# actionml/universal-recommender

Hardware: AMD Instinct MI355X
Metric: cooccurrence pairs/sec (A'A+A'B) + LLR top-k items/sec (higher is better)
Workload: dtype int32 counts / f64 LLR; 1 GPU; config4: synthetic 10M users x 2M items, Zipf-1.0, 5 event types (purchase/view/add-to-cart/search/category-pref); generator=torch Philox on the GPU (universal_recommender_amd.synth.generate_device), maxEventsPerEventType=500, maxCorrelatorsPerEventType=50, seed=20260925, entry_point=urcco_context_build_device (C ABI, include/urcco.h), launch=one process per GPU, parallelism=items range-partitioned over 1 GPU(s), one HIP stream per event type

## Files before the change

universal-recommender_amd/_lib.py:

```python
from __future__ import annotations

import ctypes as C
import os
from typing import Optional

_HERE = os.path.dirname(os.path.abspath(__file__))
DEFAULT_PATH = os.path.join(_HERE, "lib", "liburcco.so")

OK, BAD_ARG, OOM_HOST, OOM_DEVICE, HIP_ERROR, INTERNAL, NO_DEVICE, RCCL_ERROR, BUSY = range(9)
FLAG_SINGLE_STREAM = 1
FLAG_FORCE_EXCHANGE = 2
FLAG_UNORDERED_ROWS = 4
FLAG_EMULATE_RANKS = 8
UNIQUE_ID_BYTES = 128
ROW_RATE_MAHOUT_INT_DIV = 0
ROW_RATE_FRACTIONAL = 1
RNG_SPLITMIX53 = 0
RNG_MIX32 = 0x100
N_STAGES = 17
N_BINS = 7
STATS_LEN = 32
REC_MAX_CLAUSES = 16
REC_MAX_NUM = 256
REC_NO_BACKFILL = 1
# ... 4 lines not shown
REC_WEIGHT_MAX = 1 << 20
EVAL_MAX_KS = 8
EVAL_TREE_BLOCK = 256
HIST_STATS_LEN = 8
REC_LDS_LIMIT = 3072
EXCH_SIZES = 4
DBG_GATHER_ONLY = 1
DBG_NO_LLR = 2
DBG_NO_TOPK = 4
DBG_NO_SELECT = 8
DBG_NO_RANK = 16
DBG_NO_COUNT_GATHER = 512
DBG_UNFUSED_EXPAND = 4096
DBG_GATHERED_PRIMARY = 8192
DBG_UNFILTERED_EXCHANGE = 16384
DBG_SELECT_DELAY = 131072
DBG_UNPACKED_COUNTS = 1048576
DBG_NO_PREFILTER = 8388608
DBG_COUNT_SCORED = 16777216
DBG_NO_DIRECT_RANK = 33554432
DBG_COUNT_DIRECT = 67108864
DBG_NO_SMALL_WAVE = 134217728
DBG_COUNT_SMALL_WAVE = 268435456
DBG_ROW_KERNELS = DBG_GATHER_ONLY | DBG_NO_LLR | DBG_NO_TOPK | DBG_NO_SELECT | DBG_NO_RANK | DBG_NO_COUNT_GATHER | DBG_SELECT_DELAY
STAGE_NAMES = ["column_counts", "downsample_flags", "downsample_scan", "downsample_compact", "transpose", "row_work", "binning",
               "entropy", "cco_rows_micro", "cco_rows_wave", "cco_rows_block_small", "cco_rows_block", "cco_rows_cu_half", "cco_rows_cu", "cco_rows_global", "compact_indicators", "exchange"]


class UrccoError(RuntimeError):
    def __init__(self, status: int, message: str):
        super().__init__(f"liburcco: {message} (status {status})")
        self.status = status


class Csr(C.Structure):
    _fields_ = [("n_rows", C.c_int64), ("n_cols", C.c_int64), ("row_ptr", C.c_void_p), ("col_idx", C.c_void_p)]


class Dataset(C.Structure):
    _fields_ = [("matrix", Csr), ("max_elements_per_row", C.c_int32), ("max_interesting_elements", C.c_int32),
                ("min_llr", C.c_double), ("has_min_llr", C.c_int32), ("reserved", C.c_int32)]


class Options(C.Structure):
    _fields_ = [("device", C.c_int32), ("row_rate_mode", C.c_int32), ("n_gpus", C.c_int32), ("flags", C.c_int32), ("reserved", C.c_int32 * 4)]

# ... 198 lines not shown
```

universal-recommender_amd/csrc/cco_kernels.h:

```cpp
#pragma once
#include <hip/hip_runtime.h>
#include <stdint.h>

namespace urcco {

constexpr int NBINS = 7;
constexpr int MP_KMAX_HOST = 256;

constexpr int SCAN_TILE = 2048;
constexpr int DS_TILE = 4096;
constexpr int GLOBAL_BIN_BLOCKS = 128;
constexpr int BIN_TILE = 1024;
constexpr int XLX_TABLE_HOST = 4096;
constexpr int BIN_COLS_HOST = 3 * NBINS + 5;
constexpr int BIN_OFF_LEN = NBINS + 5;
constexpr int CAND_SLOTS = 64;
constexpr int STATS_LEN = 32;

constexpr int32_t DBG_GATHER_ONLY = 1;
constexpr int32_t DBG_NO_LLR = 2;
constexpr int32_t DBG_NO_TOPK = 4;
constexpr int32_t DBG_NO_SELECT = 8;
constexpr int32_t DBG_NO_RANK = 16;
constexpr int32_t DBG_NO_COUNT_GATHER = 512;
constexpr int32_t DBG_UNFUSED_EXPAND = 4096;
constexpr int32_t DBG_GATHERED_PRIMARY = 8192;
constexpr int32_t DBG_UNFILTERED_EXCHANGE = 16384;
constexpr int32_t DBG_SELECT_DELAY = 131072;
constexpr int32_t DBG_UNPACKED_COUNTS = 1048576;
constexpr int32_t DBG_NO_PREFILTER = 8388608;
constexpr int32_t DBG_COUNT_SCORED = 16777216;
constexpr int32_t DBG_NO_DIRECT_RANK = 33554432;
constexpr int32_t DBG_COUNT_DIRECT = 67108864;
constexpr int32_t DBG_NO_SMALL_WAVE = 134217728;
constexpr int32_t DBG_COUNT_SMALL_WAVE = 268435456;
constexpr int32_t DBG_ROW_KERNELS = DBG_GATHER_ONLY | DBG_NO_LLR | DBG_NO_TOPK | DBG_NO_SELECT | DBG_NO_RANK | DBG_NO_COUNT_GATHER | DBG_SELECT_DELAY;

constexpr int32_t FORM_WIDE = 1;
constexpr int32_t FORM_PS64 = 2;
constexpr int32_t FORM_TILE = 4;
constexpr int32_t FORM_PACK = 8;
constexpr int32_t FORM_HOST = 16;
constexpr unsigned long long NARROW_LIMIT = 1ull << 32;
struct ExpandForm {
  int32_t* word;
  const int32_t* pack_bad;
  int32_t host_wide;
  int32_t host_narrow;
  unsigned long long limit;
  long long seed;
};

struct CcoArgs {
  const int32_t* bin_rows;
  const int32_t* bin_off;
  const int64_t* a_col_ptr;
  const unsigned* pstart32;
  const int64_t* wp;
// ... 264 lines not shown
```

universal-recommender_amd/csrc/cco_rows.hip:

```cpp
#include "cco_kernels.h"

#include <atomic>
#include <cstdlib>

#include "cco_common.h"
#include "cco_device.h"
#include "cco_select.h"


namespace urcco {

constexpr int E0 = 1024, E1S = 4096, E1 = 8192, E2S = 16384, E2 = 32768;
constexpr int MP_KMAX = 256;

__host__ __device__ constexpr int table_slots(int E, int T) { return (2 * E / 3) / (2 * T) * (2 * T); }
constexpr int URCCO_WB1 = 512;
constexpr int URCCO_WB2 = 8192;
__device__ __forceinline__ int choose_bin(long long w, long long ca, int32_t n_cols_b, int32_t count_bits, int32_t k) {
  if (ca <= 0 || w <= 0) return -1;
  if (count_bits < 31 && ca > ((1ll << count_bits) - 1)) return NBINS - 1;
  if (w <= 64 && ca <= 64) return 0;
  int cap_bin = NBINS - 1;
  const long long dmax = (w < (long long)n_cols_b ? w : (long long)n_cols_b) * 3 + (long long)k * 3 + 2;
  if (dmax <= E0) cap_bin = 1;
  else if (dmax <= E1S) cap_bin = 2;
  else if (dmax <= E1) cap_bin = 3;
  else if (dmax <= E2S) cap_bin = 4;
  else if (dmax <= E2) cap_bin = 5;
  const int work_bin = w <= URCCO_WB1 ? 1 : (w <= URCCO_WB2 ? 2 : 4);
  return cap_bin > work_bin ? cap_bin : work_bin;
}

constexpr int MICRO_SUBS = 3;
constexpr int SMALL_SUBS = 2;
constexpr int SMALL_P0 = 2, SMALL_P1 = 4;
constexpr int SMALL_KMAX = WAVE - 1;
static_assert(SMALL_KMAX + 1 <= WAVE && SMALL_KMAX >= 1, "k + 1 survivors (a self pair among them) must fit the lanes of the fast tail");
constexpr int IBINS = NBINS - 1 + MICRO_SUBS + SMALL_SUBS;
constexpr int SPLIT_MICRO = 1, SPLIT_SMALL = 2;
__device__ __forceinline__ int micro_sub(long long w, long long ca) { return (w <= 16 && ca <= 16) ? 0 : ((w <= 32 && ca <= 32) ? 1 : 2); }
__device__ __forceinline__ int small_sub(long long w, long long ca) { return ca > WAVE ? 2 : (w <= SMALL_P0 * WAVE ? 0 : (w <= SMALL_P1 * WAVE ? 1 : 2)); }
__device__ __forceinline__ int internal_bin(int b, long long w, long long ca, int split) {
  if (b < 0) return -1;
  if (b == 0) return (split & SPLIT_MICRO) ? micro_sub(w, ca) : MICRO_SUBS - 1;
  if (b == 1) return MICRO_SUBS + ((split & SPLIT_SMALL) ? small_sub(w, ca) : SMALL_SUBS);
  return b + MICRO_SUBS - 1 + SMALL_SUBS;
}
static bool micro_split_for(int32_t n_rows) {
  static const long long min_rows = [] { const char* e = getenv("URCCO_MICRO_SPLIT_ROWS"); return e && *e ? atoll(e) : 1000000ll; }();
  return (long long)n_rows >= min_rows;
}
__host__ __device__ constexpr int internal_off_index(int ib) {
  return ib == 0 ? 0 : (ib < MICRO_SUBS ? NBINS + ib : (ib == MICRO_SUBS ? 1 : (ib <= MICRO_SUBS + SMALL_SUBS ? NBINS + ib - 1 : ib - (MICRO_SUBS - 1 + SMALL_SUBS))));
}
static_assert(internal_off_index(MICRO_SUBS + 1) == NBINS + 3 && internal_off_index(MICRO_SUBS + 2) == NBINS + 4 && internal_off_index(MICRO_SUBS + 3) == 2 &&
              internal_off_index(IBINS - 1) == NBINS - 1, "bin_off layout");
__device__ __forceinline__ int internal_start(const int32_t* __restrict__ bin_off, int ib) { return bin_off[internal_off_index(ib)]; }
constexpr int BIN_THREADS = 256;
constexpr int BIN_ITEMS = BIN_TILE / BIN_THREADS;
constexpr int BIN_COLS = IBINS + 2 * NBINS + 1;
static_assert(BIN_COLS == BIN_COLS_HOST && BIN_OFF_LEN == NBINS + MICRO_SUBS + SMALL_SUBS, "scratch sizes of the callers");

__global__ __launch_bounds__(BIN_THREADS) void bin_count_kernel(int32_t item_lo, int32_t n, const int64_t* __restrict__ work,
                                                                const int32_t* __restrict__ cnt_a, int32_t n_cols_b, int32_t count_bits, int32_t k,
                                                                int64_t* __restrict__ tile_counts, int split) {
  __shared__ long long s_acc[BIN_COLS];
  if (threadIdx.x < BIN_COLS) s_acc[threadIdx.x] = 0;
  __syncthreads();
  int c[IBINS];
  long long pw[NBINS], pu[NBINS];
#pragma unroll
  for (int k = 0; k < IBINS; ++k) c[k] = 0;
#pragma unroll
  for (int k = 0; k < NBINS; ++k) { pw[k] = 0; pu[k] = 0; }
  long long pairs = 0;
#pragma unroll
  for (int q = 0; q < BIN_ITEMS; ++q) {
    const int64_t t = (int64_t)blockIdx.x * BIN_TILE + (int64_t)threadIdx.x * BIN_ITEMS + q;
    if (t < n) {
      const long long w = work[t];
      const long long ca = cnt_a[item_lo + t];
      pairs += w;
      const int b = choose_bin(w, ca, n_cols_b, count_bits, k);
      const int ib = internal_bin(b, w, ca, split);
// ... 54 lines not shown
#pragma unroll
      for (int d = 1; d < WAVE; d <<= 1) {
        const long long o = shfl_up_i64(inc, d);
        if (lane >= d) inc += o;
      }
      if (i < n_tiles) tile_counts[i * BIN_COLS + k] = carry + inc - v;
      carry += shfl_i64(inc, WAVE - 1);
    }
    if (lane == 0) s_tot[k] = carry;
  }
  __syncthreads();
  if (threadIdx.x == 0) {
    int32_t off = 0;
    for (int ib = 0; ib < IBINS; ++ib) {
      bin_off[internal_off_index(ib)] = off;
      off += (int32_t)s_tot[ib];
    }
    bin_off[NBINS] = off;
    if (stats) {
      for (int k = 0; k < NBINS; ++k) {
        long long rows = 0;
        if (k == 0) for (int q = 0; q < MICRO_SUBS; ++q) rows += s_tot[q];
        else if (k == 1) for (int q = 0; q <= SMALL_SUBS; ++q) rows += s_tot[MICRO_SUBS + q];
        else rows = s_tot[k + MICRO_SUBS - 1 + SMALL_SUBS];
        stats[1 + k] = rows;
        stats[1 + NBINS + k] = s_tot[IBINS + k];
        stats[1 + 2 * NBINS + k] = s_tot[IBINS + NBINS + k];
      }
      stats[0] = s_tot[IBINS + 2 * NBINS];
      stats[STATS_LEN - 1] = s_tot[0] + s_tot[1];
    }
  }
}

__global__ __launch_bounds__(BIN_THREADS) void bin_scatter_kernel(int32_t item_lo, int32_t n, const int64_t* __restrict__ work,
                                                                  const int32_t* __restrict__ cnt_a, int32_t n_cols_b, int32_t count_bits, int32_t k,
                                                                  const int64_t* __restrict__ tile_counts, const int32_t* __restrict__ bin_off,
                                                                  int32_t* __restrict__ bin_rows, int split) {
  __shared__ long long s_wave[SCAN_THREADS / WAVE];
  int b[BIN_ITEMS];
#pragma unroll
  for (int q = 0; q < BIN_ITEMS; ++q) {
    const int64_t t = (int64_t)blockIdx.x * BIN_TILE + (int64_t)threadIdx.x * BIN_ITEMS + q;
    b[q] = -1;
    if (t < n) {
      const long long w = work[t], ca = cnt_a[item_lo + t];
      b[q] = internal_bin(choose_bin(w, ca, n_cols_b, count_bits, k), w, ca, split);
// ... 384 lines not shown
  __shared__ unsigned long long s_runk[MP ? 2 * MP_KMAX : 1];
  __shared__ unsigned s_runc[MP ? 2 * MP_KMAX : 1];

  const int team = TEAMS == 1 ? 0 : uni((int)threadIdx.x / T);
  const int tl = threadIdx.x % T;
  const int lane = threadIdx.x & (WAVE - 1);
  unsigned* tab = s_tab + team * E;
  unsigned* cand = tab + SH;
  unsigned long long* share = s_share + (SHARE ? team * SHARE_WORDS : 0);
  PS* ustart = reinterpret_cast<PS*>(SHARE ? reinterpret_cast<long long*>(share) : s_ustart + team * T);
  unsigned* uoff = SHARE ? reinterpret_cast<unsigned*>(share + T) : s_uoff + team * (T + 1);
  unsigned* hist = SHARE ? reinterpret_cast<unsigned*>(share) : s_hist + team * NH * 128;
  unsigned* sel_res = s_selres + team * 4;
  unsigned* nsel = sel_res + 3;
  unsigned short* lst = SHARE ? reinterpret_cast<unsigned short*>(share) + SH_LST / 2 : s_lst + team * (SEL_CAP > 0 ? SEL_CAP : 1);
  unsigned long long* amb_key = SHARE ? share : s_ambkey + team * SEL_M;
  unsigned* amb_col = SHARE ? reinterpret_cast<unsigned*>(share + SEL_M) : s_ambcol + team * SEL_M;
  unsigned long long* sel_thr = s_selthr + team * 2;
  constexpr bool PF = PK && !MP && prefilter_class(T, E);
  static_assert(!PF || !SHARE || T == WAVE || (sizeof(PS) == 4 && T * 4 + PF_BINS * 2 <= T * 8), "the histogram sits behind the 32-bit starts");
  unsigned* pfh = (SHARE && T != WAVE) ? reinterpret_cast<unsigned*>(share) + T : hist;
  constexpr unsigned DL = PF ? direct_limit(T, E) : 0u;
  static_assert(DL <= (unsigned)SEL_M, "a directly ranked row lives in the ambiguous-set arrays");
  const int list_start = (T == WAVE && PK && !MP && (bin_arg & 2048)) ? a.bin_off[NBINS + MICRO_SUBS - 1 + SMALL_SUBS] : a.bin_off[bin];
  const int list_n = a.bin_off[bin + 1] - list_start;
  const int total_teams = gridDim.x * TEAMS;
  bool ident =(long long)a.n_cols_b * 3 + (long long)a.k * 3 + 2 <= E && a.n_cols_b <= SH;
  int cb = a.count_bits;
  unsigned cmask = (1u << cb) - 1u;
  unsigned long long cand_acc = 0ull;
  const double xlx_n = *a.xlx_n;
  const bool use16 = *a.cnt16_bad == 0;

  int li = blockIdx.x * TEAMS + team;
  if (li >= list_n) return;
  const int S = total_teams;
  auto pos_of = [&](int l) { return list_start + (l < list_n ? l : list_n - 1); };
  const unsigned* wp32 = reinterpret_cast<const unsigned*>(a.wp);
  const PS* pstart;
  if constexpr (PK) pstart = a.pstart32;
  else pstart = a.pstart64;
  const int lane3 = lane < 3 ? lane : 2;
  int idv = a.bin_rows[pos_of(li + lane3 * S)];
  int64_t cs_c, ce_c;
  int64_t bnd_b;
  {
    const int id0 = (int)wave_read_lane((unsigned)idv, 0);
// ... 887 lines not shown
        cand[rank] = rc;
        kkm[rank] = rk;
      }
      wave_sync();
      settle_prefetch();
      if ((unsigned)sl < n_out) {
        out_idx[obase + sl] = (int)cand[sl];
        out_llr[obase + sl] = __longlong_as_double((long long)kkm[sl]);
      }
      if (sl == 0 && live) out_count[i - a.item_lo] = (int)n_out;
    } else {
      settle_prefetch();
    }
    i_cur = i_n1;
    i_n1 = i_n2;
    i_n2 = i_n3;
    cs1 = cs2;
    ce1 = ce2;
    wave_sync();
  }
  if (a.cand && lane == 0 && cand_acc != 0ull) atomicAdd(&a.cand[(blockIdx.x * TEAMS + team) & (CAND_SLOTS - 1)], cand_acc);
}

constexpr int SMALL_TW = 512, SMALL_LOG2TW = 9;
constexpr int SMALL_LIST = WAVE + 4;
constexpr int SMALL_WORDS = 2 * SMALL_TW;
constexpr int SMALL_FACTOR = 4;
static_assert(2 * SMALL_P1 * WAVE <= SMALL_TW && SMALL_P1 * WAVE + 2 <= SMALL_TW && 3 * SMALL_LIST <= SMALL_TW / 2 && PF_BINS / 2 <= SMALL_TW / 2, "accumulator load <= 1/2; the marks and the fallback's keys fit the phase region, its staged words and columns the accumulator");
static_assert(PF_BINS / 2 + 2 * WAVE + 3 * SMALL_LIST <= SMALL_TW && (PF_BINS / 2 + 2 * WAVE + SMALL_LIST) % 2 == 0, "fast tail arrays; 64-bit keys 8-byte aligned");
template <int P>
__global__ __launch_bounds__(256, URCCO_OCC_MICRO) void cco_rows_small_kernel(CcoArgs a, int flags) {
  if (!(a.b_packed != nullptr && (a.pk_known != 0 || *a.form == 0))) return;
  static_assert(P == SMALL_P0 || P == SMALL_P1, "one instantiation per sub-list");
  const int32_t* bin_rows = a.bin_rows;
  const int64_t* a_col_ptr = a.a_col_ptr;
  const unsigned* pstart = a.pstart32;
  const int32_t* b_col_idx = a.b_packed;
  const int cshift = 32 - a.count_bits;
  const unsigned colmask = (1u << cshift) - 1u;
  const int32_t* cnt_a = a.cnt_a;
  const double* ent_a = a.ent_a;
  const double* xlx_tab = a.xlx_tab;
  const double* xlx_hi = a.xlx_hi;
  const double* col_ent = a.col_ent;
  int32_t* out_idx = a.out_idx;
  double* out_llr = a.out_llr;
  int32_t* out_count = a.out_count;
  const long long n_users = a.n_users;
  const bool has_pf = a.pf_limit != nullptr;
  const unsigned short* lim_tab = has_pf ? a.pf_limit : reinterpret_cast<const unsigned short*>(a.cnt_a);
  constexpr int TEAMS = 256 / WAVE;
  __shared__ __attribute__((aligned(16))) unsigned s_tab[TEAMS * SMALL_WORDS];
  const int team = threadIdx.x / WAVE;
  const int lane = threadIdx.x & (WAVE - 1);
  unsigned* tab = s_tab + team * SMALL_WORDS;
  unsigned* marks = tab + SMALL_TW;
  unsigned* pfh = marks;
  unsigned* st_v = marks + PF_BINS / 2;
  unsigned* st_c = st_v + WAVE;
  unsigned* cand = st_c + WAVE;
  unsigned long long* kkm = reinterpret_cast<unsigned long long*>(cand + SMALL_LIST);
  unsigned long long* fkeys = reinterpret_cast<unsigned long long*>(marks);
  const int list_start = P == SMALL_P0 ? a.bin_off[1] : a.bin_off[NBINS + 3];
  const int list_n = (P == SMALL_P0 ? a.bin_off[NBINS + 3] : a.bin_off[NBINS + 4]) - list_start;
  const int total_teams = gridDim.x * TEAMS;
  const bool ident = a.n_cols_b <= SMALL_TW;
  const int cb = a.count_bits;
  const unsigned cmask = (1u << cb) - 1u;
  const double xlx_n = __longlong_as_double((long long)uni((int64_t)__double_as_longlong(*a.xlx_n)));
  const unsigned pf_need = (unsigned)a.k + (a.exclude_self ? 1u : 0u);
  unsigned long long cand_acc = 0ull;

  int li = blockIdx.x * TEAMS + team;
  if (li >= list_n) return;
  const int stride = total_teams;
  auto pos_of = [&](int l) { return list_start + (l < list_n ? l : list_n - 1); };
  const unsigned* wp32 = reinterpret_cast<const unsigned*>(a.wp);
  const int lane3 = lane < 3 ? lane : 2;
  int idv = bin_rows[pos_of(li + lane3 * stride)];
  int64_t bnd_b;
  unsigned pf_w1, pf_wp, pf_start;
  int n_cur;
  {
    const int id0 = (int)wave_read_lane((unsigned)idv, 0);
    const int id1 = (int)wave_read_lane((unsigned)idv, 1);
    const int64_t cs0 = uni(a_col_ptr[id0]), ce0 = uni(a_col_ptr[id0 + 1]);
    bnd_b = a_col_ptr[id1 + (lane & 1)];
    n_cur = (int)(ce0 - cs0);
    const int64_t pl = lane < n_cur ? cs0 + lane : ce0 - 1;
    pf_w1 = wp32[ce0];
    pf_wp = wp32[pl];
    pf_start = pstart[pl];
  }
  URCCO_SETTLE(idv); URCCO_SETTLE(bnd_b); URCCO_SETTLE(pf_w1); URCCO_SETTLE(pf_wp); URCCO_SETTLE(pf_start);
#pragma unroll
  for (int q = 0; q < SMALL_TW / WAVE; ++q) tab[lane + q * WAVE] = 0u;
  int64_t bnd_c = 0;
  for (; li < list_n; li += stride, bnd_b = bnd_c) {
    const int i = (int)wave_read_lane((unsigned)idv, 0);
    const int id2 = (int)wave_read_lane((unsigned)idv, 2);
    const int64_t cs_n = wave_read_lane64(bnd_b, 0), ce_n = wave_read_lane64(bnd_b, 1);
    const unsigned w0 = wave_read_lane(pf_wp, 0);
    unsigned total = uni(pf_w1) - w0;
    if (total > (unsigned)(P * WAVE) || n_cur > WAVE) {
      if (lane == 0) atomicAdd(a.err, 1ull);
      total = 0u;
    }
    const bool owns_user = lane < n_cur;
    const unsigned my_off = owns_user ? pf_wp - w0 : total;
    const unsigned my_delta = (owns_user ? pf_start : 0u) - my_off;
    int lz = lane;
    URCCO_OPAQUE(lz);
    idv = bin_rows[pos_of(li + (1 + (lz < 3 ? lz : 2)) * stride)];
    bnd_c = a_col_ptr[id2 + (lz & 1)];
    int iv = i;
    URCCO_OPAQUE(iv);
    const int row_ca = cnt_a[iv];
    const double row_entropy = ent_a[iv];
    const unsigned row_lim = lim_tab[iv];
    n_cur = (int)(ce_n - cs_n);
    {
      const int64_t pl = lz < n_cur ? cs_n + lz : ce_n - 1;
      pf_w1 = wp32[ce_n];
      pf_wp = wp32[pl];
      pf_start = pstart[pl];
    }
#pragma unroll
    for (int r = 0; r < P; ++r) marks[lane + r * WAVE] = 0u;
    if (lane < 2) marks[P * WAVE + lane] = 0u;
    wave_sync();
    if (owns_user && my_off <= total) atomicMax(&marks[my_off], (unsigned)lane);
    wave_sync();
    unsigned jj[P];
    unsigned carry = 0u;
#pragma unroll
    for (int r = 0; r < P; ++r) {
      const unsigned m = wave_inclusive_max(marks[lane + r * WAVE]);
      const unsigned o = m > carry ? m : carry;
      carry = wave_read_lane(o, WAVE - 1);
      const unsigned base_o = wave_gather(my_delta, o);
      const unsigned t = (unsigned)(r * WAVE + lane);
      jj[r] = 0u;
      if (t < total) jj[r] = (unsigned)b_col_idx[base_o + t];
    }
    unsigned slot[P];
#pragma unroll
    for (int r = 0; r < P; ++r) {
      slot[r] = 0xffffffffu;
      if ((unsigned)(r * WAVE + lane) < total) {
        bool ok;
        slot[r] = tab_insert_claim(tab, (jj[r] & colmask) + 1u, cb, (unsigned)(SMALL_TW - 1), 32 - SMALL_LOG2TW, ident, &ok);
        if (!ok) atomicAdd(a.err, 1ull);
      }
    }
    wave_sync();
    unsigned vv[P];
    unsigned D = 0u;
#pragma unroll
    for (int r = 0; r < P; ++r) {
      const bool is_cand = slot[r] != 0xffffffffu;
      D += (unsigned)__popcll(__ballot(is_cand));
      vv[r] = 0u;
      if (is_cand) {
        vv[r] = tab[slot[r]];
        tab[slot[r]] = 0u;
      }
    }
    if (has_pf && D > pf_need) {
      unsigned zero = 0u;
      URCCO_OPAQUE(zero);
      *reinterpret_cast<uint2*>(&pfh[2 * lane]) = make_uint2(zero, zero);
      wave_sync();
#pragma unroll
      for (int r = 0; r < P; ++r)
        if (vv[r] != 0u) pf_count(pfh, vv[r] & cmask, jj[r] >> cshift);
      wave_sync();
      unsigned cstar, lim;
      if (pf_find_cut(pfh, lane, pf_need, row_lim, cstar, lim)) {
#pragma unroll
        for (int r = 0; r < P; ++r)
          if (pf_drops(vv[r] & cmask, jj[r] >> cshift, cstar, lim)) vv[r] = 0u;
      }
      wave_sync();
    }
    unsigned pos[P];
    unsigned n_surv = 0u;
#pragma unroll
    for (int r = 0; r < P; ++r) {
      const unsigned long long m = __ballot(vv[r] != 0u);
      pos[r] = n_surv + lanes_below(m);
      n_surv += (unsigned)__popcll(m);
    }
    if (!(flags & 4096)) cand_acc += (flags & 256) ? n_surv : D;
    else cand_acc += n_surv <= (unsigned)WAVE ? 1ull : (1ull << 32) + 1ull;
    const int64_t obase = ((int64_t)(i - a.item_lo)) * a.k;
    auto settle_prefetch = [&]() {
      URCCO_SETTLE(idv); URCCO_SETTLE(bnd_c); URCCO_SETTLE(pf_w1); URCCO_SETTLE(pf_wp); URCCO_SETTLE(pf_start);
    };
    const bool fast = n_surv <= (unsigned)WAVE;
    {
      unsigned* sv = fast ? st_v : tab;
      unsigned* sc = fast ? st_c : tab + SMALL_TW / 2;
#pragma unroll
      for (int r = 0; r < P; ++r)
        if (vv[r] != 0u) {
          sv[pos[r]] = vv[r];
          sc[pos[r]] = jj[r] >> cshift;
        }
    }
    unsigned* cand_l = cand;
    unsigned long long* kkm_l = kkm;
    unsigned n_list = n_surv;
    bool listed = true;
    unsigned long long mk = 0ull;
    int jc = 0;
    if (fast) {
      wave_sync();
      const bool is_cand = (unsigned)lane < n_surv;
      const unsigned v1 = is_cand ? st_v[lane] : 0u;
      const unsigned cbj = is_cand ? st_c[lane] : 0u;
      if (n_surv + (unsigned)lane < (unsigned)SMALL_LIST) {
        unsigned zero = 0u;
        URCCO_OPAQUE(zero);
        *reinterpret_cast<uint2*>(&kkm[n_surv + (unsigned)lane]) = make_uint2(zero, zero);
        cand[n_surv + (unsigned)lane] = 0xffffffffu;
      }
      jc = (int)(v1 >> cb) - 1;
      const long long k11 = (long long)(v1 & cmask);
      const bool in_tables = !is_cand || llr_operands_in_tables((unsigned)k11, (long long)row_ca, cbj, n_users, col_ent);
      const bool all_in_tables = __ballot(!in_tables) == 0ull;
      if (is_cand) {
        if (!(a.exclude_self && jc == i)) {
          const double llr = all_in_tables ? llr_from_tables(row_entropy, xlx_n, (unsigned)k11, (unsigned)row_ca, cbj, xlx_tab, xlx_hi, col_ent)
                                           : llr_of(row_entropy, xlx_n, k11, (long long)row_ca, (long long)cbj, n_users, xlx_tab, xlx_hi, col_ent);
          if (llr > 0.0 && (!a.has_min_llr || llr >= a.min_llr)) mk = (unsigned long long)__double_as_longlong(llr);
        }
        kkm[lane] = mk;
        cand[lane] = (unsigned)jc;
      }
      wave_sync();
    } else {
      unsigned* fcol = tab + SMALL_TW / 2;
      wave_sync();
      unsigned n_valid = 0u;
      unsigned long long kand = ~0ull, kor = 0ull;
#pragma unroll 1
      for (unsigned base = 0; base < n_surv; base += WAVE) {
        const unsigned x = base + (unsigned)lane;
        unsigned long long key = 0ull;
        if (x < n_surv) {
          const unsigned v1 = tab[x], cbj = fcol[x];
          const int j = (int)(v1 >> cb) - 1;
          const long long k11 = (long long)(v1 & cmask);
          if (!(a.exclude_self && j == i)) {
            const double llr = llr_operands_in_tables((unsigned)k11, (long long)row_ca, cbj, n_users, col_ent)
                                   ? llr_from_tables(row_entropy, xlx_n, (unsigned)k11, (unsigned)row_ca, cbj, xlx_tab, xlx_hi, col_ent)
                                   : llr_of(row_entropy, xlx_n, k11, (long long)row_ca, (long long)cbj, n_users, xlx_tab, xlx_hi, col_ent);
            if (llr > 0.0 && (!a.has_min_llr || llr >= a.min_llr)) key = (unsigned long long)__double_as_longlong(llr);
          }
          fkeys[x] = key;
          fcol[x] = (unsigned)j;
        }
        if (key != 0ull) {
          kand &= key;
          kor |= key;
// ... 109 lines not shown
        } else {
          rk = kkm_l[ln];
          rc = cand_l[ln];
          rank = rank_by_counting_strided<1>(kkm_l, cand_l, 0u, n_list, rk, rc);
        }
        wave_sync();
        const unsigned n_out = (unsigned)(n_valid < a.k ? n_valid : a.k);
        if ((unsigned)lane < n_list && rk != 0ull && rank < n_out) {
          cand_l[rank] = rc;
          kkm_l[rank] = rk;
        }
        wave_sync();
        settle_prefetch();
        if ((unsigned)lane < n_out) {
          out_idx[obase + lane] = (int)cand_l[lane];
          out_llr[obase + lane] = __longlong_as_double((long long)kkm_l[lane]);
        }
        if (lane == 0) out_count[i - a.item_lo] = (int)n_out;
      }
    }
    if (!fast) {
      wave_sync();
#pragma unroll
      for (int q = 0; q < SMALL_TW / WAVE; ++q) tab[lane + q * WAVE] = 0u;
    }
    wave_sync();
  }
  if (a.cand && cand_acc != 0ull && lanes_below(~0ull) == 0u) atomicAdd(&a.cand[blockIdx.x & (CAND_SLOTS - 1)], cand_acc);
}

constexpr int GB_THREADS = 1024;
constexpr int GSEL_K = 1024;

__device__ __forceinline__ int64_t g_start(const unsigned* ps32, const int64_t* ps64, bool nar, int64_t p) { return nar ? (int64_t)ps32[p] : ps64[p]; }
__device__ __forceinline__ int64_t g_len(const int64_t* wp, bool nar, int64_t p) {
  const unsigned* w = reinterpret_cast<const unsigned*>(wp);
  return nar ? (int64_t)(unsigned)(w[p + 1] - w[p]) : wp[p + 1] - wp[p];
}
__global__ __launch_bounds__(GB_THREADS) void cco_rows_global_kernel(CcoArgs a) {
  constexpr int NW = GB_THREADS / WAVE;
  __shared__ unsigned long long s_pkey[2][NW];
  __shared__ int s_pcol[2][NW];
  __shared__ int s_ncand;
  __shared__ SelScratch s_select;
  __shared__ int s_nsel;
  __shared__ unsigned long long s_selk[GSEL_K];
  __shared__ unsigned s_selc[GSEL_K];
// ... 166 lines not shown
template <int T, int E, int U, bool MP = false>
constexpr RowClass row_class(int factor) {
  return {T < 256 ? 256 : T, (T < 256 ? 256 : T) / T, factor, MP ? 0u : direct_limit(T, E),
          cco_rows_kernel<T, E, U, MP, true, false>, cco_rows_kernel<T, E, U, MP, false, true>, cco_rows_kernel<T, E, U, MP, false, false>};
}
constexpr RowClass ROW_CLASS[NBINS] = {{256, 4, 8, 0u, nullptr, nullptr, nullptr},
                                       row_class<64, E0, URCCO_U_WAVE>(8),         row_class<256, E1S, URCCO_U_BS>(8), row_class<256, E1, URCCO_U_B>(8),
                                       row_class<512, E2S, URCCO_U_H>(4),          row_class<1024, E2, URCCO_U_C>(4),  row_class<1024, E2, URCCO_U_C, true>(2)};
constexpr int MICRO_FACTOR32 = 3, MICRO_FACTOR16 = 2;

static int blocks_per_cu(int bin) {
  static std::atomic<int> cache[NBINS];
  if (cache[bin].load(std::memory_order_relaxed) == 0) {
    int n = 0;
    const hipError_t e = bin == 0 ? hipOccupancyMaxActiveBlocksPerMultiprocessor(&n, (cco_rows_micro_kernel<WAVE, false, false>), ROW_CLASS[0].block, 0)
                                  : hipOccupancyMaxActiveBlocksPerMultiprocessor(&n, ROW_CLASS[bin].plain, ROW_CLASS[bin].block, 0);
    cache[bin].store((e == hipSuccess && n > 0) ? n : 1, std::memory_order_relaxed);
  }
  return cache[bin].load(std::memory_order_relaxed);
}

hipError_t launch_cco_rows_bin(hipStream_t st, int n_cu, const CcoArgs& args, RowsPlan plan, int bin, int32_t n_rows) {
  const RowClass& c = ROW_CLASS[bin];
  auto grid = [&](int factor) {
    const long long fill = (long long)n_cu * blocks_per_cu(bin);
    long long cap = ((long long)n_rows + c.teams * 32 - 1) / (c.teams * 32);
    if (cap < 2 * fill) cap = 2 * fill;
    long long blocks = fill * factor;
    if (blocks > cap) blocks = cap;
    return dim3((unsigned)blocks);
  };
  const bool count_direct = (args.debug & DBG_COUNT_DIRECT) != 0, count_small = (args.debug & DBG_COUNT_SMALL_WAVE) != 0;
  CcoArgs pk = args, plain = args, small = args;
  if ((count_direct && c.direct == 0u) || count_small) pk.cand = nullptr;
  if (count_direct || count_small) plain.cand = nullptr;
  if (count_direct) small.cand = nullptr;
  const int pk_bits = ((args.debug & DBG_COUNT_SCORED) ? 256 : 0) | ((args.debug & DBG_NO_DIRECT_RANK) ? 512 : 0) | (count_direct ? 1024 : 0);
  auto enqueue = [&](auto dbg_kernel, auto pk_kernel, auto plain_kernel, int factor, auto... bin_arg) {
    if (plan == RowsPlan::DEBUG) hipLaunchKernelGGL(dbg_kernel, grid(factor), dim3(c.block), 0, st, plain, bin_arg...);
    if (plan_runs_pk(plan)) hipLaunchKernelGGL(pk_kernel, grid(factor), dim3(c.block), 0, st, pk, (bin_arg | pk_bits)...);
    if (plan_runs_plain(plan)) hipLaunchKernelGGL(plain_kernel, grid(factor), dim3(c.block), 0, st, plain, bin_arg...);
  };
  if (bin == 0) {
    enqueue(cco_rows_micro_kernel<64, true, false>, cco_rows_micro_kernel<64, false, true>, cco_rows_micro_kernel<64, false, false>, c.factor);
    if (micro_split_for(n_rows)) {
      enqueue(cco_rows_micro_kernel<32, true, false>, cco_rows_micro_kernel<32, false, true>, cco_rows_micro_kernel<32, false, false>, MICRO_FACTOR32);
      enqueue(cco_rows_micro_kernel<16, true, false>, cco_rows_micro_kernel<16, false, true>, cco_rows_micro_kernel<16, false, false>, MICRO_FACTOR16);
    }
  } else if (bin == NBINS - 1 && args.g_blocks > 0) {
    plain.b_packed = nullptr;
    hipLaunchKernelGGL(cco_rows_global_kernel, dim3((unsigned)args.g_blocks), dim3(GB_THREADS), 0, st, plain);
  } else if (bin == 1 && plan_runs_pk(plan) && micro_split_for(n_rows) && args.k <= SMALL_KMAX && !(args.debug & DBG_NO_SMALL_WAVE)) {
    const int small_bits = ((args.debug & DBG_COUNT_SCORED) ? 256 : 0) | (count_small ? 4096 : 0);
    hipLaunchKernelGGL(cco_rows_small_kernel<SMALL_P0>, grid(SMALL_FACTOR), dim3(c.block), 0, st, small, small_bits);
    hipLaunchKernelGGL(cco_rows_small_kernel<SMALL_P1>, grid(SMALL_FACTOR), dim3(c.block), 0, st, small, small_bits);
    hipLaunchKernelGGL(c.pk, grid(c.factor), dim3(c.block), 0, st, pk, bin | pk_bits | 2048);
    if (plan_runs_plain(plan)) hipLaunchKernelGGL(c.plain, grid(c.factor), dim3(c.block), 0, st, plain, bin);
  } else {
    enqueue(c.dbg, c.pk, c.plain, c.factor, bin);
  }
  return hipGetLastError();
}

__global__ __launch_bounds__(256) void bin_out_stats_kernel(const int32_t* __restrict__ bin_rows, const int32_t* __restrict__ bin_off,
                                                            int32_t item_lo, const int32_t* __restrict__ out_count, const unsigned long long* __restrict__ cand,
                                                            int64_t* __restrict__ stats) {
  __shared__ long long s_wave[SCAN_THREADS / WAVE];
  const int bin = blockIdx.x;
  if (bin == 0 && blockIdx.y == 0 && threadIdx.x == 0 && cand) {
    long long c = 0;
    for (int q = 0; q < CAND_SLOTS; ++q) c += (long long)cand[q];
    stats[2 + 4 * NBINS] = c;
  }
  long long v = 0;
  for (int t = bin_off[bin] + blockIdx.y * 256 + threadIdx.x; t < bin_off[bin + 1]; t += 256 * gridDim.y) v += out_count[bin_rows[t] - item_lo];
  long long tot;
  block_exclusive_scan(v, s_wave, &tot);
  if (threadIdx.x == 0 && tot) atomicAdd((unsigned long long*)&stats[1 + 3 * NBINS + bin], (unsigned long long)tot);
// ... 10 lines not shown
```

Measured before the change: 39.83 billion pairs/s.

## Route mid-size rows to a one-wave kernel with two users per lane

```diff
diff --git a/universal-recommender_amd/_lib.py b/universal-recommender_amd/_lib.py
--- a/universal-recommender_amd/_lib.py
+++ b/universal-recommender_amd/_lib.py
@@ -50,6 +50,8 @@
 DBG_COUNT_DIRECT = 67108864
 DBG_NO_SMALL_WAVE = 134217728
 DBG_COUNT_SMALL_WAVE = 268435456
+DBG_NO_BLOCK_SMALL_WAVE = 536870912
+DBG_COUNT_BLOCK_SMALL_WAVE = 1073741824
 DBG_ROW_KERNELS = DBG_GATHER_ONLY | DBG_NO_LLR | DBG_NO_TOPK | DBG_NO_SELECT | DBG_NO_RANK | DBG_NO_COUNT_GATHER | DBG_SELECT_DELAY
 STAGE_NAMES = ["column_counts", "downsample_flags", "downsample_scan", "downsample_compact", "transpose", "row_work", "binning",
                "entropy", "cco_rows_micro", "cco_rows_wave", "cco_rows_block_small", "cco_rows_block", "cco_rows_cu_half", "cco_rows_cu", "cco_rows_global", "compact_indicators", "exchange"]
diff --git a/universal-recommender_amd/csrc/cco_kernels.h b/universal-recommender_amd/csrc/cco_kernels.h
--- a/universal-recommender_amd/csrc/cco_kernels.h
+++ b/universal-recommender_amd/csrc/cco_kernels.h
@@ -12,8 +12,8 @@
 constexpr int GLOBAL_BIN_BLOCKS = 128;
 constexpr int BIN_TILE = 1024;
 constexpr int XLX_TABLE_HOST = 4096;
-constexpr int BIN_COLS_HOST = 3 * NBINS + 5;
-constexpr int BIN_OFF_LEN = NBINS + 5;
+constexpr int BIN_COLS_HOST = 3 * NBINS + 7;
+constexpr int BIN_OFF_LEN = NBINS + 7;
 constexpr int CAND_SLOTS = 64;
 constexpr int STATS_LEN = 32;
 
@@ -34,6 +34,8 @@
 constexpr int32_t DBG_COUNT_DIRECT = 67108864;
 constexpr int32_t DBG_NO_SMALL_WAVE = 134217728;
 constexpr int32_t DBG_COUNT_SMALL_WAVE = 268435456;
+constexpr int32_t DBG_NO_BLOCK_SMALL_WAVE = 536870912;
+constexpr int32_t DBG_COUNT_BLOCK_SMALL_WAVE = 1073741824;
 constexpr int32_t DBG_ROW_KERNELS = DBG_GATHER_ONLY | DBG_NO_LLR | DBG_NO_TOPK | DBG_NO_SELECT | DBG_NO_RANK | DBG_NO_COUNT_GATHER | DBG_SELECT_DELAY;
 
 constexpr int32_t FORM_WIDE = 1;
diff --git a/universal-recommender_amd/csrc/cco_rows.hip b/universal-recommender_amd/csrc/cco_rows.hip
--- a/universal-recommender_amd/csrc/cco_rows.hip
+++ b/universal-recommender_amd/csrc/cco_rows.hip
@@ -32,34 +32,48 @@
 }
 
 constexpr int MICRO_SUBS = 3;
-constexpr int SMALL_SUBS = 2;
-constexpr int SMALL_P0 = 2, SMALL_P1 = 4;
+constexpr int SMALL_SUBS = 3;
+constexpr int BLOCK_SUBS = 1;
+constexpr int SMALL_P0 = 2, SMALL_P1 = 4, SMALL_P2 = 8;
+constexpr int SMALL_U2 = 2;
 constexpr int SMALL_KMAX = WAVE - 1;
 static_assert(SMALL_KMAX + 1 <= WAVE && SMALL_KMAX >= 1, "k + 1 survivors (a self pair among them) must fit the lanes of the fast tail");
-constexpr int IBINS = NBINS - 1 + MICRO_SUBS + SMALL_SUBS;
+static_assert(SMALL_P2 * WAVE >= URCCO_WB1, "every row of the one-wave class fits eight pairs per lane");
+constexpr int IBINS = NBINS - 1 + MICRO_SUBS + SMALL_SUBS + BLOCK_SUBS;
 constexpr int SPLIT_MICRO = 1, SPLIT_SMALL = 2;
 __device__ __forceinline__ int micro_sub(long long w, long long ca) { return (w <= 16 && ca <= 16) ? 0 : ((w <= 32 && ca <= 32) ? 1 : 2); }
-__device__ __forceinline__ int small_sub(long long w, long long ca) { return ca > WAVE ? 2 : (w <= SMALL_P0 * WAVE ? 0 : (w <= SMALL_P1 * WAVE ? 1 : 2)); }
+__device__ __forceinline__ int small_sub(long long w, long long ca) {
+  return ca > SMALL_U2 * WAVE ? 3 : ((ca > WAVE || w > SMALL_P1 * WAVE) ? 2 : (w <= SMALL_P0 * WAVE ? 0 : 1));
+}
+__device__ __forceinline__ int block_sub(long long w, long long ca) { return (ca <= SMALL_U2 * WAVE && w <= SMALL_P2 * WAVE) ? 0 : 1; }
 __device__ __forceinline__ int internal_bin(int b, long long w, long long ca, int split) {
   if (b < 0) return -1;
   if (b == 0) return (split & SPLIT_MICRO) ? micro_sub(w, ca) : MICRO_SUBS - 1;
   if (b == 1) return MICRO_SUBS + ((split & SPLIT_SMALL) ? small_sub(w, ca) : SMALL_SUBS);
-  return b + MICRO_SUBS - 1 + SMALL_SUBS;
+  if (b == 2) return MICRO_SUBS + SMALL_SUBS + 1 + ((split & SPLIT_SMALL) ? block_sub(w, ca) : BLOCK_SUBS);
+  return b + MICRO_SUBS - 1 + SMALL_SUBS + BLOCK_SUBS;
 }
 static bool micro_split_for(int32_t n_rows) {
   static const long long min_rows = [] { const char* e = getenv("URCCO_MICRO_SPLIT_ROWS"); return e && *e ? atoll(e) : 1000000ll; }();
   return (long long)n_rows >= min_rows;
 }
 __host__ __device__ constexpr int internal_off_index(int ib) {
-  return ib == 0 ? 0 : (ib < MICRO_SUBS ? NBINS + ib : (ib == MICRO_SUBS ? 1 : (ib <= MICRO_SUBS + SMALL_SUBS ? NBINS + ib - 1 : ib - (MICRO_SUBS - 1 + SMALL_SUBS))));
-}
-static_assert(internal_off_index(MICRO_SUBS + 1) == NBINS + 3 && internal_off_index(MICRO_SUBS + 2) == NBINS + 4 && internal_off_index(MICRO_SUBS + 3) == 2 &&
-              internal_off_index(IBINS - 1) == NBINS - 1, "bin_off layout");
+  constexpr int B2 = MICRO_SUBS + SMALL_SUBS + 1;
+  return ib == 0 ? 0
+                 : (ib < MICRO_SUBS ? NBINS + ib
+                                    : (ib == MICRO_SUBS ? 1
+                                                        : (ib < B2 ? NBINS + ib - 1
+                                                                   : (ib == B2 ? 2 : (ib <= B2 + BLOCK_SUBS ? NBINS + ib - 2 : ib - (MICRO_SUBS - 1 + SMALL_SUBS + BLOCK_SUBS))))));
+}
+constexpr int OFF_SMALL_P1 = NBINS + 3, OFF_SMALL_U2 = NBINS + 4, OFF_WAVE_REST = NBINS + 5, OFF_BLOCK_REST = NBINS + 6;
+static_assert(internal_off_index(MICRO_SUBS + 1) == OFF_SMALL_P1 && internal_off_index(MICRO_SUBS + 2) == OFF_SMALL_U2 && internal_off_index(MICRO_SUBS + 3) == OFF_WAVE_REST &&
+              internal_off_index(MICRO_SUBS + 4) == 2 && internal_off_index(MICRO_SUBS + 5) == OFF_BLOCK_REST && internal_off_index(MICRO_SUBS + 6) == 3 &&
+              internal_off_index(IBINS - 1) == NBINS - 1 && OFF_BLOCK_REST == BIN_OFF_LEN - 1, "bin_off layout");
 __device__ __forceinline__ int internal_start(const int32_t* __restrict__ bin_off, int ib) { return bin_off[internal_off_index(ib)]; }
 constexpr int BIN_THREADS = 256;
 constexpr int BIN_ITEMS = BIN_TILE / BIN_THREADS;
 constexpr int BIN_COLS = IBINS + 2 * NBINS + 1;
-static_assert(BIN_COLS == BIN_COLS_HOST && BIN_OFF_LEN == NBINS + MICRO_SUBS + SMALL_SUBS, "scratch sizes of the callers");
+static_assert(BIN_COLS == BIN_COLS_HOST && BIN_OFF_LEN == NBINS + MICRO_SUBS + SMALL_SUBS + BLOCK_SUBS, "scratch sizes of the callers");
 
 __global__ __launch_bounds__(BIN_THREADS) void bin_count_kernel(int32_t item_lo, int32_t n, const int64_t* __restrict__ work,
                                                                 const int32_t* __restrict__ cnt_a, int32_t n_cols_b, int32_t count_bits, int32_t k,
@@ -160,7 +174,8 @@
         long long rows = 0;
         if (k == 0) for (int q = 0; q < MICRO_SUBS; ++q) rows += s_tot[q];
         else if (k == 1) for (int q = 0; q <= SMALL_SUBS; ++q) rows += s_tot[MICRO_SUBS + q];
-        else rows = s_tot[k + MICRO_SUBS - 1 + SMALL_SUBS];
+        else if (k == 2) for (int q = 0; q <= BLOCK_SUBS; ++q) rows += s_tot[MICRO_SUBS + SMALL_SUBS + 1 + q];
+        else rows = s_tot[k + MICRO_SUBS - 1 + SMALL_SUBS + BLOCK_SUBS];
         stats[1 + k] = rows;
         stats[1 + NBINS + k] = s_tot[IBINS + k];
         stats[1 + 2 * NBINS + k] = s_tot[IBINS + NBINS + k];
@@ -591,7 +606,8 @@
   unsigned* pfh = (SHARE && T != WAVE) ? reinterpret_cast<unsigned*>(share) + T : hist;
   constexpr unsigned DL = PF ? direct_limit(T, E) : 0u;
   static_assert(DL <= (unsigned)SEL_M, "a directly ranked row lives in the ambiguous-set arrays");
-  const int list_start = (T == WAVE && PK && !MP && (bin_arg & 2048)) ? a.bin_off[NBINS + MICRO_SUBS - 1 + SMALL_SUBS] : a.bin_off[bin];
+  const int list_start = (T == WAVE && PK && !MP && (bin_arg & 2048)) ? a.bin_off[(bin_arg & 8192) ? OFF_SMALL_U2 : OFF_WAVE_REST]
+                         : ((T == 256 && E == E1S && PK && !MP && (bin_arg & 2048)) ? a.bin_off[OFF_BLOCK_REST] : a.bin_off[bin]);
   const int list_n = a.bin_off[bin + 1] - list_start;
   const int total_teams = gridDim.x * TEAMS;
   bool ident =(long long)a.n_cols_b * 3 + (long long)a.k * 3 + 2 <= E && a.n_cols_b <= SH;
@@ -1525,16 +1541,21 @@
   if (a.cand && lane == 0 && cand_acc != 0ull) atomicAdd(&a.cand[(blockIdx.x * TEAMS + team) & (CAND_SLOTS - 1)], cand_acc);
 }
 
-constexpr int SMALL_TW = 512, SMALL_LOG2TW = 9;
+__host__ __device__ constexpr int small_log2tw(int P) { return P <= SMALL_P1 ? 9 : 10; }
 constexpr int SMALL_LIST = WAVE + 4;
-constexpr int SMALL_WORDS = 2 * SMALL_TW;
 constexpr int SMALL_FACTOR = 4;
-static_assert(2 * SMALL_P1 * WAVE <= SMALL_TW && SMALL_P1 * WAVE + 2 <= SMALL_TW && 3 * SMALL_LIST <= SMALL_TW / 2 && PF_BINS / 2 <= SMALL_TW / 2, "accumulator load <= 1/2; the marks and the fallback's keys fit the phase region, its staged words and columns the accumulator");
-static_assert(PF_BINS / 2 + 2 * WAVE + 3 * SMALL_LIST <= SMALL_TW && (PF_BINS / 2 + 2 * WAVE + SMALL_LIST) % 2 == 0, "fast tail arrays; 64-bit keys 8-byte aligned");
-template <int P>
-__global__ __launch_bounds__(256, URCCO_OCC_MICRO) void cco_rows_small_kernel(CcoArgs a, int flags) {
+constexpr int SMALL_OCC_P2 = 5;
+template <int P, int UPL>
+__global__ __launch_bounds__(256, (P == SMALL_P2 ? SMALL_OCC_P2 : URCCO_OCC_MICRO)) void cco_rows_small_kernel(CcoArgs a, int flags) {
   if (!(a.b_packed != nullptr && (a.pk_known != 0 || *a.form == 0))) return;
-  static_assert(P == SMALL_P0 || P == SMALL_P1, "one instantiation per sub-list");
+  static_assert(((P == SMALL_P0 || P == SMALL_P1) && UPL == 1) || (P == SMALL_P2 && UPL == SMALL_U2), "one instantiation per sub-list shape");
+  constexpr int LOG2TW = small_log2tw(P), TW = 1 << LOG2TW, WORDS = 2 * TW;
+  constexpr int MAX_USERS = UPL * WAVE;
+  static_assert(2 * P * WAVE <= TW && P * WAVE + 2 <= TW && 3 * SMALL_LIST <= TW / 2 && PF_BINS / 2 <= TW / 2,
+                "accumulator load <= 1/2; the marks and the fallback's keys (64 P of 64 bits) fit the phase region, its staged words and columns (64 P each) the accumulator");
+  static_assert(PF_BINS / 2 + 2 * WAVE + 3 * SMALL_LIST <= TW && (PF_BINS / 2 + 2 * WAVE + SMALL_LIST) % 2 == 0, "fast tail arrays; 64-bit keys 8-byte aligned");
+  static_assert(P * WAVE < 65536 && MAX_USERS <= 128, "the fallback's digit histogram and the prefilter's count 64 P candidates in 16-bit fields; a mark carries a user index");
+  static_assert((256 / WAVE) * WORDS * 4 <=160 * 1024 / (P == SMALL_P2 ? SMALL_OCC_P2 : URCCO_OCC_MICRO), "LDS per block at the occupancy the kernel is compiled for");
   const int32_t* bin_rows = a.bin_rows;
   const int64_t* a_col_ptr = a.a_col_ptr;
   const unsigned* pstart = a.pstart32;
@@ -1553,21 +1574,22 @@
   const bool has_pf = a.pf_limit != nullptr;
   const unsigned short* lim_tab = has_pf ? a.pf_limit : reinterpret_cast<const unsigned short*>(a.cnt_a);
   constexpr int TEAMS = 256 / WAVE;
-  __shared__ __attribute__((aligned(16))) unsigned s_tab[TEAMS * SMALL_WORDS];
+  __shared__ __attribute__((aligned(16))) unsigned s_tab[TEAMS * WORDS];
   const int team = threadIdx.x / WAVE;
   const int lane = threadIdx.x & (WAVE - 1);
-  unsigned* tab = s_tab + team * SMALL_WORDS;
-  unsigned* marks = tab + SMALL_TW;
+  unsigned* tab = s_tab + team * WORDS;
+  unsigned* marks = tab + TW;
   unsigned* pfh = marks;
   unsigned* st_v = marks + PF_BINS / 2;
   unsigned* st_c = st_v + WAVE;
   unsigned* cand = st_c + WAVE;
   unsigned long long* kkm = reinterpret_cast<unsigned long long*>(cand + SMALL_LIST);
   unsigned long long* fkeys = reinterpret_cast<unsigned long long*>(marks);
-  const int list_start = P == SMALL_P0 ? a.bin_off[1] : a.bin_off[NBINS + 3];
-  const int list_n = (P == SMALL_P0 ? a.bin_off[NBINS + 3] : a.bin_off[NBINS + 4]) - list_start;
+  const bool of_block = P == SMALL_P2 && (flags & 8192);
+  const int list_start = a.bin_off[P == SMALL_P0 ? 1 : (P == SMALL_P1 ? OFF_SMALL_P1 : (of_block ? 2 : OFF_SMALL_U2))];
+  const int list_n = a.bin_off[P == SMALL_P0 ? OFF_SMALL_P1 : (P == SMALL_P1 ? OFF_SMALL_U2 : (of_block ? OFF_BLOCK_REST : OFF_WAVE_REST))] - list_start;
   const int total_teams = gridDim.x * TEAMS;
-  const bool ident = a.n_cols_b <= SMALL_TW;
+  const bool ident = a.n_cols_b <= TW;
   const int cb = a.count_bits;
   const unsigned cmask = (1u << cb) - 1u;
   const double xlx_n = __longlong_as_double((long long)uni((int64_t)__double_as_longlong(*a.xlx_n)));
@@ -1582,7 +1604,7 @@
   const int lane3 = lane < 3 ? lane : 2;
   int idv = bin_rows[pos_of(li + lane3 * stride)];
   int64_t bnd_b;
-  unsigned pf_w1, pf_wp, pf_start;
+  unsigned pf_w1, pf_wp[UPL], pf_start[UPL];
   int n_cur;
   {
     const int id0 = (int)wave_read_lane((unsigned)idv, 0);
@@ -1590,28 +1612,38 @@
     const int64_t cs0 = uni(a_col_ptr[id0]), ce0 = uni(a_col_ptr[id0 + 1]);
     bnd_b = a_col_ptr[id1 + (lane & 1)];
     n_cur = (int)(ce0 - cs0);
-    const int64_t pl = lane < n_cur ? cs0 + lane : ce0 - 1;
     pf_w1 = wp32[ce0];
-    pf_wp = wp32[pl];
-    pf_start = pstart[pl];
-  }
-  URCCO_SETTLE(idv); URCCO_SETTLE(bnd_b); URCCO_SETTLE(pf_w1); URCCO_SETTLE(pf_wp); URCCO_SETTLE(pf_start);
-#pragma unroll
-  for (int q = 0; q < SMALL_TW / WAVE; ++q) tab[lane + q * WAVE] = 0u;
+#pragma unroll
+    for (int q = 0; q < UPL; ++q) {
+      const int64_t pl = lane + q * WAVE < n_cur ? cs0 + lane + q * WAVE : ce0 - 1;
+      pf_wp[q] = wp32[pl];
+      pf_start[q] = pstart[pl];
+    }
+  }
+  URCCO_SETTLE(idv); URCCO_SETTLE(bnd_b); URCCO_SETTLE(pf_w1);
+#pragma unroll
+  for (int q = 0; q < UPL; ++q) { URCCO_SETTLE(pf_wp[q]); URCCO_SETTLE(pf_start[q]); }
+#pragma unroll
+  for (int q = 0; q < TW / WAVE; ++q) tab[lane + q * WAVE] = 0u;
   int64_t bnd_c = 0;
   for (; li < list_n; li += stride, bnd_b = bnd_c) {
     const int i = (int)wave_read_lane((unsigned)idv, 0);
     const int id2 = (int)wave_read_lane((unsigned)idv, 2);
     const int64_t cs_n = wave_read_lane64(bnd_b, 0), ce_n = wave_read_lane64(bnd_b, 1);
-    const unsigned w0 = wave_read_lane(pf_wp, 0);
+    const unsigned w0 = wave_read_lane(pf_wp[0], 0);
     unsigned total = uni(pf_w1) - w0;
-    if (total > (unsigned)(P * WAVE) || n_cur > WAVE) {
+    if (total > (unsigned)(P * WAVE) || n_cur > MAX_USERS) {
       if (lane == 0) atomicAdd(a.err, 1ull);
       total = 0u;
     }
-    const bool owns_user = lane < n_cur;
-    const unsigned my_off = owns_user ? pf_wp - w0 : total;
-    const unsigned my_delta = (owns_user ? pf_start : 0u) - my_off;
+    bool owns_user[UPL];
+    unsigned my_off[UPL], my_delta[UPL];
+#pragma unroll
+    for (int q = 0; q < UPL; ++q) {
+      owns_user[q] = lane + q * WAVE < n_cur;
+      my_off[q] = owns_user[q] ? pf_wp[q] - w0 : total;
+      my_delta[q] = (owns_user[q] ? pf_start[q] : 0u) - my_off[q];
+    }
     int lz = lane;
     URCCO_OPAQUE(lz);
     idv = bin_rows[pos_of(li + (1 + (lz < 3 ? lz : 2)) * stride)];
@@ -1622,17 +1654,20 @@
     const double row_entropy = ent_a[iv];
     const unsigned row_lim = lim_tab[iv];
     n_cur = (int)(ce_n - cs_n);
-    {
-      const int64_t pl = lz < n_cur ? cs_n + lz : ce_n - 1;
-      pf_w1 = wp32[ce_n];
-      pf_wp = wp32[pl];
-      pf_start = pstart[pl];
+    pf_w1 = wp32[ce_n];
+#pragma unroll
+    for (int q = 0; q < UPL; ++q) {
+      const int64_t pl = lz + q * WAVE < n_cur ? cs_n + lz + q * WAVE : ce_n - 1;
+      pf_wp[q] = wp32[pl];
+      pf_start[q] = pstart[pl];
     }
 #pragma unroll
     for (int r = 0; r < P; ++r) marks[lane + r * WAVE] = 0u;
     if (lane < 2) marks[P * WAVE + lane] = 0u;
     wave_sync();
-    if (owns_user && my_off <= total) atomicMax(&marks[my_off], (unsigned)lane);
+#pragma unroll
+    for (int q = 0; q < UPL; ++q)
+      if (owns_user[q] && my_off[q] <= total) atomicMax(&marks[my_off[q]], (unsigned)(lane + q * WAVE));
     wave_sync();
     unsigned jj[P];
     unsigned carry = 0u;
@@ -1641,7 +1676,15 @@
       const unsigned m = wave_inclusive_max(marks[lane + r * WAVE]);
       const unsigned o = m > carry ? m : carry;
       carry = wave_read_lane(o, WAVE - 1);
-      const unsigned base_o = wave_gather(my_delta, o);
+      unsigned base_o;
+      if constexpr (UPL == 1) {
+        base_o = wave_gather(my_delta[0], o);
+      } else {
+        const unsigned src = o & (unsigned)(WAVE - 1);
+        const unsigned d0 = wave_gather(my_delta[0], src);
+        const unsigned d1 = wave_gather(my_delta[1], src);
+        base_o = o < (unsigned)WAVE ? d0 : d1;
+      }
       const unsigned t = (unsigned)(r * WAVE + lane);
       jj[r] = 0u;
       if (t < total) jj[r] = (unsigned)b_col_idx[base_o + t];
@@ -1652,7 +1695,7 @@
       slot[r] = 0xffffffffu;
       if ((unsigned)(r * WAVE + lane) < total) {
         bool ok;
-        slot[r] = tab_insert_claim(tab, (jj[r] & colmask) + 1u, cb, (unsigned)(SMALL_TW - 1), 32 - SMALL_LOG2TW, ident, &ok);
+        slot[r] = tab_insert_claim(tab, (jj[r] & colmask) + 1u, cb, (unsigned)(TW - 1), 32 - LOG2TW, ident, &ok);
         if (!ok) atomicAdd(a.err, 1ull);
       }
     }
@@ -1698,12 +1741,14 @@
     else cand_acc += n_surv <= (unsigned)WAVE ? 1ull : (1ull << 32) + 1ull;
     const int64_t obase = ((int64_t)(i - a.item_lo)) * a.k;
     auto settle_prefetch = [&]() {
-      URCCO_SETTLE(idv); URCCO_SETTLE(bnd_c); URCCO_SETTLE(pf_w1); URCCO_SETTLE(pf_wp); URCCO_SETTLE(pf_start);
+      URCCO_SETTLE(idv); URCCO_SETTLE(bnd_c); URCCO_SETTLE(pf_w1);
+#pragma unroll
+      for (int q = 0; q < UPL; ++q) { URCCO_SETTLE(pf_wp[q]); URCCO_SETTLE(pf_start[q]); }
     };
     const bool fast = n_surv <= (unsigned)WAVE;
     {
       unsigned* sv = fast ? st_v : tab;
-      unsigned* sc = fast ? st_c : tab + SMALL_TW / 2;
+      unsigned* sc = fast ? st_c : tab + TW / 2;
 #pragma unroll
       for (int r = 0; r < P; ++r)
         if (vv[r] != 0u) {
@@ -1743,7 +1788,7 @@
       }
       wave_sync();
     } else {
-      unsigned* fcol = tab + SMALL_TW / 2;
+      unsigned* fcol = tab + TW / 2;
       wave_sync();
       unsigned n_valid = 0u;
       unsigned long long kand = ~0ull, kor = 0ull;
@@ -1899,7 +1944,7 @@
     if (!fast) {
       wave_sync();
 #pragma unroll
-      for (int q = 0; q < SMALL_TW / WAVE; ++q) tab[lane + q * WAVE] = 0u;
+      for (int q = 0; q < TW / WAVE; ++q) tab[lane + q * WAVE] = 0u;
     }
     wave_sync();
   }
@@ -2112,8 +2157,8 @@
 
 hipError_t launch_cco_rows_bin(hipStream_t st, int n_cu, const CcoArgs& args, RowsPlan plan, int bin, int32_t n_rows) {
   const RowClass& c = ROW_CLASS[bin];
-  auto grid = [&](int factor) {
-    const long long fill = (long long)n_cu * blocks_per_cu(bin);
+  auto grid = [&](int factor, int per_cu = 0) {
+    const long long fill = (long long)n_cu * (per_cu > 0 ? per_cu : blocks_per_cu(bin));
     long long cap = ((long long)n_rows + c.teams * 32 - 1) / (c.teams * 32);
     if (cap < 2 * fill) cap = 2 * fill;
     long long blocks = fill * factor;
@@ -2121,10 +2166,19 @@
     return dim3((unsigned)blocks);
   };
   const bool count_direct = (args.debug & DBG_COUNT_DIRECT) != 0, count_small = (args.debug & DBG_COUNT_SMALL_WAVE) != 0;
-  CcoArgs pk = args, plain = args, small = args;
-  if ((count_direct && c.direct == 0u) || count_small) pk.cand = nullptr;
-  if (count_direct || count_small) plain.cand = nullptr;
-  if (count_direct) small.cand = nullptr;
+  const bool count_block = (args.debug & DBG_COUNT_BLOCK_SMALL_WAVE) != 0;
+  CcoArgs pk = args, plain = args, small = args, small2 = args;
+  if ((count_direct && c.direct == 0u) || count_small || count_block) pk.cand = nullptr;
+  if (count_direct || count_small || count_block) plain.cand = nullptr;
+  if (count_direct || count_block) small.cand = nullptr;
+  if (count_direct || count_small) small2.cand = nullptr;
+  if (count_block) {
+    const char* only = getenv("URCCO_COUNT_BLOCK_LIST");
+    if (only && *only && atoi(only) != bin) small2.cand = nullptr;
+  }
+  const bool small_split = plan_runs_pk(plan) && micro_split_for(n_rows) && args.k <= SMALL_KMAX;
+  const bool block_small = small_split && !(args.debug & DBG_NO_BLOCK_SMALL_WAVE);
+  const int small2_bits = ((args.debug & DBG_COUNT_SCORED) ? 256 : 0) | (count_block ? 4096 : 0);
   const int pk_bits = ((args.debug & DBG_COUNT_SCORED) ? 256 : 0) | ((args.debug & DBG_NO_DIRECT_RANK) ? 512 : 0) | (count_direct ? 1024 : 0);
   auto enqueue = [&](auto dbg_kernel, auto pk_kernel, auto plain_kernel, int factor, auto... bin_arg) {
     if (plan == RowsPlan::DEBUG) hipLaunchKernelGGL(dbg_kernel, grid(factor), dim3(c.block), 0, st, plain, bin_arg...);
@@ -2140,10 +2194,15 @@
   } else if (bin == NBINS - 1 && args.g_blocks > 0) {
     plain.b_packed = nullptr;
     hipLaunchKernelGGL(cco_rows_global_kernel, dim3((unsigned)args.g_blocks), dim3(GB_THREADS), 0, st, plain);
-  } else if (bin == 1 && plan_runs_pk(plan) && micro_split_for(n_rows) && args.k <= SMALL_KMAX && !(args.debug & DBG_NO_SMALL_WAVE)) {
+  } else if (bin == 1 && small_split && !(args.debug & DBG_NO_SMALL_WAVE)) {
     const int small_bits = ((args.debug & DBG_COUNT_SCORED) ? 256 : 0) | (count_small ? 4096 : 0);
-    hipLaunchKernelGGL(cco_rows_small_kernel<SMALL_P0>, grid(SMALL_FACTOR), dim3(c.block), 0, st, small, small_bits);
-    hipLaunchKernelGGL(cco_rows_small_kernel<SMALL_P1>, grid(SMALL_FACTOR), dim3(c.block), 0, st, small, small_bits);
+    hipLaunchKernelGGL((cco_rows_small_kernel<SMALL_P0, 1>), grid(SMALL_FACTOR), dim3(c.block), 0, st, small, small_bits);
+    hipLaunchKernelGGL((cco_rows_small_kernel<SMALL_P1, 1>), grid(SMALL_FACTOR), dim3(c.block), 0, st, small, small_bits);
+    if (block_small) hipLaunchKernelGGL((cco_rows_small_kernel<SMALL_P2, SMALL_U2>), grid(SMALL_FACTOR, SMALL_OCC_P2), dim3(c.block), 0, st, small2, small2_bits);
+    hipLaunchKernelGGL(c.pk, grid(c.factor), dim3(c.block), 0, st, pk, bin | pk_bits | 2048 | (block_small ? 0 : 8192));
+    if (plan_runs_plain(plan)) hipLaunchKernelGGL(c.plain, grid(c.factor), dim3(c.block), 0, st, plain, bin);
+  } else if (bin == 2 && block_small && !count_direct) {
+    hipLaunchKernelGGL((cco_rows_small_kernel<SMALL_P2, SMALL_U2>), grid(SMALL_FACTOR, SMALL_OCC_P2), dim3(256), 0, st, small2, small2_bits | 8192);
     hipLaunchKernelGGL(c.pk, grid(c.factor), dim3(c.block), 0, st, pk, bin | pk_bits | 2048);
     if (plan_runs_plain(plan)) hipLaunchKernelGGL(c.plain, grid(c.factor), dim3(c.block), 0, st, plain, bin);
   } else {
```

After: 40.91 billion pairs/s, median of 6. +2.7%, better.
